# xipengwang/AprilSAM

Measured on NVIDIA H100. Metric: Gauss-Newton solves/sec (batch + incremental) on M3500 & 100k-pose graph, higher is better.
Workload: dtype f64

## Files before the change

aprilsam_b200/csrc/asam_kernels.cuh:

```cuda
#pragma once

#include <cuda_runtime.h>

#include <cstdint>

#include "asam_cuda.h"

#define ASAM_TR_FLAG (1 << 30)
#define ASAM_MAX_CACHED_CHILDREN 24

__device__ __forceinline__ double d_mod2pi(double v)
{
    const double twopi = 6.2831853071795862319959;
    const double pi = 3.141592653589793238462643383279502884196;
    double w = v + pi;
    return (w - twopi * floor(w / twopi)) - pi;
}

__device__ __forceinline__ void d_atb(const double *A, const double *B, double *C)
{
#pragma unroll
    for (int i = 0; i < 3; i++)
#pragma unroll
        for (int j = 0; j < 3; j++) {
// ... 1216 lines not shown
                    ok = 0;
                    break;
                }
            }
            __threadfence();
            *s_flag = ok;
        }
        __syncthreads();
        if (!*s_flag)
            return false;
        for (int e = tid; e < ASAM_TPB * ASAM_TPB; e += nt) {
            const int ii = e % ASAM_TPB, j = e / ASAM_TPB;
            D[e] = (ii >= j && ii < pb && j < pb) ? __ldcg(&F[(k0 + ii) + (size_t) (k0 + j) * ld]) : 0.0;
        }
        for (int e = tid; e < ASAM_TPB; e += nt)
            rdv[e] = e < pb ? __ldcg(&dinv[k0 + e]) : 0.0;
        __syncthreads();
        if (row)
            trsm_row(Li, D, rdv, pb, F + i + (size_t) k0 * ld, ld, Wnext ? Wnext + (size_t) i * ASAM_LDW : nullptr);
        return true;
    };

    {
        const int pb = min(ASAM_TPB, c);
        if (trow && tid == 0)
            t_mark = d_now();
        const int nchunk = (m + 1 + ASAM_TROWS - 1) / ASAM_TROWS;
        bool first = true;
        for (int ch = w; ch < nchunk || first; ch += G) {
            panel(0, pb, ch < nchunk ? ch * ASAM_TROWS : -1);
            first = false;
        }
        if (!team_barrier(tc, s_flag))
            return false;
        if (trow && tid == 0)
            t_panel += d_now() - t_mark;
        if (w == 0)
            writeback(0, pb);
    }
    int seq = 0;
    const bool pt_on = a.ptrace && s == a.ptrace_sn && w < 8 && tid == 0;
    for (int k0 = 0; k0 < c; k0 += ASAM_TPB) {
        unsigned long long *pt = (pt_on && k0 / ASAM_TPB < a.ptrace_panels) ? a.ptrace + ((size_t) (k0 / ASAM_TPB) * 8 + w) * 8 : nullptr;
        if (pt) {
            pt[0] = d_now();
            pt[1] = pt[2] = pt[3] = pt[0];
            pt[5] = (unsigned long long) m;
            pt[6] = (unsigned long long) G;
        }
        const int pb = min(ASAM_TPB, c - k0);
        const int kn0 = k0 + pb;
        const bool has_next = kn0 < c;
        const int pbn = has_next ? min(ASAM_TPB, c - kn0) : 0;
        const int ncrew = has_next ? 1 + (m - (kn0 + pbn) + 1 + ASAM_CROWS - 1) / ASAM_CROWS : 0;
        ++seq;
        if (w < ncrew) {
            if (trow && tid == 0)
                t_mark = d_now();
            if (w == 0) {
                __syncthreads();
                for (int e = tid; e < ASAM_TPB * ASAM_TPB; e += nt)
                    D[e] = 0.0;
                tile(k0, pb, kn0, pbn, kn0, pbn, D);
                if (pt)
                    pt[1] = d_now();
                diag_publish(kn0, pbn, seq);
                if (pt)
                    pt[2] = d_now();
            }
            if (v3) {
                for (int it = (w == 0 ? G : w); it < ncrew; it += G) {
                    const int rb0 = kn0 + pbn + (it - 1) * ASAM_CROWS;
                    tile_rm<2>(F, ld, Wbuf(k0 / ASAM_TPB), (pb + 3) & ~3, kn0, pbn, rb0, min(ASAM_CROWS, m - rb0 + 1), 2, Li, Li,
                               Lj3, mbar, mb_parity);
                    if (pt && w > 0 && it == w)
                        pt[1] = d_now();
                    if (!rows_solve_staged(kn0, pbn, rb0, seq, Wbuf(kn0 / ASAM_TPB)))
                        return false;
                }
            } else {
                for (int it = (w == 0 ? G : w); it < ncrew; it += G) {
                    const int rb0 = kn0 + pbn + (it - 1) * ASAM_CROWS;
                    tile(k0, pb, kn0, pbn, rb0, min(ASAM_CROWS, m - rb0 + 1), nullptr);
                }
                if (pt && w > 0)
                    pt[1] = d_now();
                for (int it = (w == 0 ? G : w); it < ncrew; it += G) {
                    const int rb0 = kn0 + pbn + (it - 1) * ASAM_CROWS;
                    if (!rows_solve(kn0, pbn, rb0, seq, nullptr))
                        return false;
                }
            }
            if (pt && w > 0)
                pt[2] = d_now();
            if (trow && tid == 0)
                t_panel += d_now() - t_mark;
        }

        const int j0 = kn0 + pbn;
        const int nfree = (G - ncrew >= 2) ? G - ncrew : G, wfree = (G - ncrew >= 2) ? w - ncrew : w;
        int n256 = 0;
        for (int cb0 = j0; cb0 < m; cb0 += ASAM_TCOLS)
            n256 += (m - cb0 + 1 + 255) / 256;
        const int TR = (n256 < 2 * nfree) ? 128 : 256;
        if (wfree >= 0) {
            int u = 0;
            for (int cb0 = j0; cb0 < m; cb0 += ASAM_TCOLS)
                for (int rb0 = cb0; rb0 <= m; rb0 += TR, ++u)
                    if (u % nfree == wfree)
                        tile(k0, pb, cb0, min(ASAM_TCOLS, m - cb0), rb0, min(TR, m - rb0 + 1), nullptr);
        }
        if (pt)
            pt[3] = d_now();
        if (!team_barrier(tc, s_flag))
            return false;
        if (pt) {
            pt[4] = d_now();
            pt[7] = (unsigned long long) ncrew;
        }
    }
    if (w == 0 && tid == 0)
        atomicExch(crew_bar, 0);

    if (trow && tid == 0) {
        trow[4] = d_now();
        trow[7] = (unsigned long long) (unsigned) m | (t_panel << 32);
    }
    if (w == 0) {
        for (int e = tid; e < c; e += nt)
            a.y[3 * (size_t) d.first + e] = __ldcg(&F[m + (size_t) e * ld]);
        __syncthreads();
        if (tid == 0 && d.parent >= 0) {
            __threadfence();
            atomicAdd(&a.arrive[d.parent], 1);
        }
    }
    team_leave(tc);
    __syncthreads();
    return true;
}

__device__ __forceinline__ void ticket_release(int *ticket, int *done)
{
    __syncthreads();
    if (threadIdx.x == 0) {
        __threadfence();
        if (atomicAdd(done, 1) == (int) gridDim.x - 1) {
            atomicExch(ticket, 0);
            atomicExch(done, 0);
        }
    }
}

__device__ bool cta_front(const FacArgs &a, const int t, const int s, const int nw, const asam_sn_desc_t &d, double *sm,
                          asam_sn_desc_t *s_cd, int *s_abort, unsigned long long tr0, const int keepw = 0)
{
    const int tid = threadIdx.x, nt = blockDim.x;
    const int lane = tid & 31, warp = tid >> 5, nwarps = nt >> 5;
    int *err = a.ctrl + 1;
    unsigned long long tr1 = 0, tr2 = 0, tr3 = 0, tr4 = 0, accA = 0, accB = 0;
    const int m = 3 * d.mb, c = 3 * d.cb, ld = ASAM_LD(m);
    const int *seg = a.ipool + d.seg;
    const int *children = seg + 2 * d.mb;
    const int *a_slot = children + d.ch_cnt;
    const int *a_rb = a_slot + d.a_cnt;
    const int *a_cb = a_rb + d.a_cnt;
    double *Fg = a.arena + d.f_off;
    const long long fsz = (long long) ld * m;
    const bool use_sm = fsz + (ld + 1) / 2 + 2 <= (long long) a.smem_doubles;
    double *F = use_sm ? sm : Fg;
    int *dmap = (int *) (sm + (use_sm ? fsz : 0));
    double *Pbuf = sm + (ld + 1) / 2 + 1;
    double *dinv = a.dinv + 3 * (size_t) d.first;

    if (use_sm) {
        for (int i = tid; i < (int) fsz; i += nt)
            F[i] = 0.0;
    } else {
        for (int j = warp; j < m; j += nwarps)
            for (int i = j + lane; i <= m; i += 32)
                F[i + (size_t) j * ld] = 0.0;
    }
    for (int e = tid; e < d.ch_cnt && e < ASAM_MAX_CACHED_CHILDREN; e += nt)
        s_cd[e] = a.sn[children[e]];
    __syncthreads();
    __shared__ int s_doff[ASAM_MAX_CACHED_CHILDREN + 1];
    bool dmap_ahead = false;
    if (use_sm && g_dmap_ahead && d.ch_cnt > 0 && d.ch_cnt <= ASAM_MAX_CACHED_CHILDREN) {
        if (tid == 0) {
            int o = 0;
            for (int e = 0; e < d.ch_cnt; e++) {
                s_doff[e] = o;
                o += 3 * (s_cd[e].mb - s_cd[e].cb) + 1;
            }
            s_doff[d.ch_cnt] = o;
        }
        __syncthreads();
        dmap_ahead = (long long) s_doff[d.ch_cnt] <= 2 * ((long long) a.smem_doubles - fsz) - 2;
        if (dmap_ahead)
            for (int ci = 0; ci < d.ch_cnt; ++ci) {
                const int cc = 3 * s_cd[ci].cb, cr = 3 * s_cd[ci].mb - cc;
                const int *crel = a.ipool + s_cd[ci].seg + s_cd[ci].mb;
                int *dm = dmap + s_doff[ci];
                for (int i = tid; i <= cr; i += nt)
                    dm[i] = (i < cr) ? 3 * crel[(cc + i) / 3] + (cc + i) % 3 : m;
            }
    }
    for (int e = tid; e < d.cb * 9; e += nt) {
        int k = e / 9, p = (e % 9) / 3, q = e % 3;
        if (p >= q)
            F[(3 * k + p) + (size_t) (3 * k + q) * ld] =
                a.Adiag[9 * (size_t) a.q2node[d.first + k] + q * 3 + p];
    }
    for (int e = tid; e < c; e += nt)
        F[m + (size_t) e * ld] = a.Bq[3 * (size_t) a.q2node[d.first + e / 3] + e % 3];
    for (int e = tid; e < d.a_cnt * 9; e += nt) {
        int i = e / 9, p = (e % 9) / 3, q = e % 3;
        const int rbf = a_rb[i];
        const int rb = rbf & ~ASAM_TR_FLAG;
        const int si = (rbf & ASAM_TR_FLAG) ? (p * 3 + q) : (q * 3 + p);
        F[(3 * rb + p) + (size_t) (3 * a_cb[i] + q) * ld] = a.Aoff[9 * (size_t) a_slot[i] + si];
    }
    if (a.trace && tid == 0)
        tr1 = d_now();

    if (nw > 0 && tid == 0) {
        SpinClock spins;
        while (ld_volatile(&a.arrive[s]) < nw) {
            __nanosleep(32);
            if (spin_over(spins, a.spin_limit) || ld_volatile(err) < 0) {
                atomicCAS(err, 0, -(1 + s));
                *s_abort = 1;
                break;
            }
        }
        a.arrive[s] = 0;
        __threadfence();
    }
    __syncthreads();
    if (*s_abort)
        return false;
    if (a.trace && tid == 0)
        tr2 = d_now();

    for (int ci = 0; ci < d.ch_cnt; ++ci) {
        const asam_sn_desc_t cd = ci < ASAM_MAX_CACHED_CHILDREN ? s_cd[ci] : a.sn[children[ci]];
        const int cm = 3 * cd.mb, cc = 3 * cd.cb, cr = cm - cc, cld = ASAM_LD(cm);
        const double *CF = a.arena + cd.f_off;
        const int *crel = a.ipool + cd.seg + cd.mb;
        if (dmap_ahead) {
            dmap = (int *) (sm + fsz) + s_doff[ci];
        } else {
            for (int i = tid; i <= cr; i += nt)
                dmap[i] = (i < cr) ? 3 * crel[(cc + i) / 3] + (cc + i) % 3 : m;
            __syncthreads();
        }
        if (use_sm && cr <= 159) {
            for (int j0 = warp; j0 < cr; j0 += 4 * nwarps) {
                double v[4][5];
#pragma unroll
                for (int q = 0; q < 4; q++) {
                    const int j = j0 + q * nwarps;
                    const double *ccol = CF + (size_t) (cc + min(j, cr - 1)) * cld + cc;
#pragma unroll
                    for (int u = 0; u < 5; u++) {
                        const int i = j + lane + 32 * u;
                        v[q][u] = (j < cr && i <= cr) ? __ldcg(ccol + i) : 0.0;
                    }
                }
#pragma unroll
                for (int q = 0; q < 4; q++) {
                    const int j = j0 + q * nwarps;
                    if (j < cr) {
                        double *fcol = F + (size_t) dmap[j] * ld;
#pragma unroll
                        for (int u = 0; u < 5; u++) {
                            const int i = j + lane + 32 * u;
                            if (i <= cr)
                                fcol[dmap[i]] += v[q][u];
                        }
                    }
                }
            }
        } else {
            for (int j = warp; j < cr; j += nwarps) {
                const double *ccol = CF + (size_t) (cc + j) * cld + cc;
                double *fcol = F + (size_t) dmap[j] * ld;
                for (int i0 = j + lane; i0 <= cr; i0 += 256) {
                    double v[8], dv[8];
                    int di[8];
#pragma unroll
                    for (int u = 0; u < 8; u++) {
                        const bool ok = i0 + 32 * u <= cr;
                        v[u] = ok ? __ldcg(ccol + i0 + 32 * u) : 0.0;
                        di[u] = ok ? dmap[i0 + 32 * u] : -1;
                    }
#pragma unroll
                    for (int u = 0; u < 8; u++)
                        dv[u] = di[u] >= 0 ? fcol[di[u]] : 0.0;
#pragma unroll
                    for (int u = 0; u < 8; u++)
                        if (di[u] >= 0)
                            fcol[di[u]] = dv[u] + v[u];
                }
            }
        }
        __syncthreads();
    }
    if (a.trace && tid == 0)
        tr3 = d_now();

    int kstart = 0;
    if (use_sm && keepw != 0) {
        const int keep = 3 * (keepw >> 16), m_old = 3 * (keepw & 0xffff), ld_old = ASAM_LD(m_old);
        if (keep > 0 && keep < c && m_old <= m && keep <= m_old) {
            for (int j = warp; j < keep; j += nwarps) {
                const double *oc = Fg + (size_t) j * ld_old;
                double *nc = F + (size_t) j * ld;
                for (int i = j + lane; i < m; i += 32)
                    nc[i] = i < m_old ? oc[i] : 0.0;
                if (lane == 0)
                    nc[m] = oc[m_old];
            }
            __syncthreads();
            if (a.smem_mma)
                trailing_update_mma(F, ld, F, ld, keep, keep, m, m);
            else
                trailing_update<2, 8>(F, ld, F, ld, keep, keep, m, m);
            __syncthreads();
            kstart = keep;
        }
    }
    if (use_sm) {
        const int pbw = a.pb_smem;
        for (int k0 = kstart; k0 < c; k0 += pbw) {
            const int pb = min(pbw, c - k0);
            double *P = F + (size_t) k0 * ld;
            unsigned long long ta = 0, tb = 0;
            if (a.trace && tid == 0)
                ta = d_now();
            panel_factor(P, ld, k0, pb, m, s, err, dinv);
            if (a.trace && tid == 0) {
                tb = d_now();
                accA += tb - ta;
            }
            const int n = m - (k0 + pb);
            if (a.smem_mma >= 2 && n > 0)
                trailing_update_mma(F, ld, P, ld, pb, k0 + pb, m, m);
            else if (n > 48)
                trailing_update<2, 8>(F, ld, P, ld, pb, k0 + pb, m, m);
            else
                trailing_update<1, 4>(F, ld, P, ld, pb, k0 + pb, m, m);
            __syncthreads();
        }
    } else {
        const int avail = a.smem_doubles - ((ld + 1) / 2 + 2);
        int PB = avail / ld;
        PB = PB > a.solo_pb ? a.solo_pb : PB;
        PB = PB >= ASAM_PB ? PB - (PB % ASAM_PB) : PB - (PB % 3);
        if (PB < 3) {
            if (tid == 0)
                atomicCAS(err, 0, -(1 + s));
            return false;
        }
        for (int k0 = 0; k0 < c; k0 += PB) {
            const int pbw = min(PB, c - k0);
            for (int p = warp; p < pbw; p += nwarps)
                for (int i = k0 + lane; i <= m; i += 32)
                    Pbuf[i + (size_t) p * ld] = F[i + (size_t) (k0 + p) * ld];
            __syncthreads();
            double *Cp = Pbuf - (size_t) k0 * ld;
            for (int k1 = 0; k1 < pbw; k1 += ASAM_PB) {
                const int pb = min(ASAM_PB, pbw - k1);
                panel_factor(Pbuf + (size_t) k1 * ld, ld, k0 + k1, pb, m, s, err, dinv);
                if (k1 + pb < pbw) {
                    trailing_update<2, 8>(Cp, ld, Pbuf + (size_t) k1 * ld, ld, pb, k0 + k1 + pb, k0 + pbw, m);
                    __syncthreads();
                }
            }
            for (int p = warp; p < pbw; p += nwarps)
                for (int i = k0 + lane; i <= m; i += 32)
                    F[i + (size_t) (k0 + p) * ld] = Pbuf[i + (size_t) p * ld];
            trailing_update<4, 8>(F, ld, Pbuf, ld, pbw, k0 + pbw, m, m);
            __syncthreads();
        }
    }
    if (a.trace && tid == 0)
        tr4 = d_now();

    if (use_sm) {
        for (int j = c + warp; j < m; j += nwarps)
            for (int i = j + lane; i <= m; i += 32)
                Fg[i + (size_t) j * ld] = F[i + (size_t) j * ld];
    }
    __syncthreads();
    if (tid == 0 && d.parent >= 0) {
        __threadfence();
        atomicAdd(&a.arrive[d.parent], 1);
    }
    for (int e = tid; e < c; e += nt)
        a.y[3 * (size_t) d.first + e] = F[m + (size_t) e * ld];
    if (use_sm) {
        for (int j = warp; j < c; j += nwarps)
            for (int i = j + lane; i <= m; i += 32)
                Fg[i + (size_t) j * ld] = F[i + (size_t) j * ld];
    }
    __syncthreads();
    if (tid == 0) {
        if (a.trace) {
            unsigned smid;
            asm volatile("mov.u32 %0, %%smid;" : "=r"(smid));
            unsigned long long *tr = a.trace + 8 * (size_t) t;
            tr[0] = tr0; tr[1] = tr1; tr[2] = tr2; tr[3] = tr3; tr[4] = tr4; tr[5] = d_now();
            (void) smid;
            tr[6] = (unsigned long long) s | (accB << 32);
            tr[7] = (unsigned long long) (unsigned) m | (accA << 32);
        }
    }
    __syncthreads();
    return true;
}

__global__ void __launch_bounds__(256, 1) k_factor(FacArgs a)
{
    extern __shared__ __align__(16) double sm[];
    __shared__ int s_task, s_abort;
    __shared__ asam_sn_desc_t s_cd[ASAM_MAX_CACHED_CHILDREN];
    __shared__ __align__(8) unsigned long long s_mbar;
    const int tid = threadIdx.x;
    unsigned mb_parity = 0;
    if (tid == 0)
        mbar_init(&s_mbar, 1);
    __syncthreads();
    for (;;) {
        if (tid == 0) {
            s_task = atomicAdd(&a.ctrl[0], 1);
            s_abort = 0;
        }
        __syncthreads();
        const int t = s_task;
        if (t >= a.ntasks)
            break;
        unsigned long long tr0 = 0;
        if (a.trace && tid == 0)
            tr0 = d_now();
        const int s = a.tasks[t];
        const int nwp = a.nwait[t];
        const int nw = nwp & 0xffff, tw = (nwp >> 16) & 0xff, tG = (nwp >> 24) & 0x7f;
        const asam_sn_desc_t d = a.sn[s];
        if (tG >= 1) {
            unsigned long long *trow = (a.trace && tw == 0) ? a.trace + 8 * (size_t) t : nullptr;
            if (trow && tid == 0) {
                trow[0] = tr0; trow[1] = tr0;
            }
            if (!team_front(a, d, s, nw, tw, tG, sm, &s_abort, trow, &s_mbar, mb_parity))
                break;
            if (a.trace && tid == 0) {
                unsigned long long *tr = a.trace + 8 * (size_t) t;
                if (tw == 0) {
                    tr[5] = d_now();
                    tr[6] = (unsigned long long) s | ((unsigned long long) tG << 32);
                } else {
                    tr[0] = tr0; tr[1] = tr0; tr[2] = tr0; tr[3] = tr0; tr[4] = d_now(); tr[5] = tr[4];
                    tr[6] = (unsigned long long) s | ((unsigned long long) tG << 32);
                    tr[7] = (unsigned long long) (unsigned) (3 * d.mb);
                }
            }
            __syncthreads();
            continue;
        }
        if (!cta_front(a, t, s, nw, d, sm, s_cd, &s_abort, tr0, a.keep ? a.keep[t] : 0))
            break;
    }
    ticket_release(&a.ctrl[0], &a.ctrl[3]);
}

#define ASAM_LEAF_M 63
#define ASAM_LEAF_WARPS 7
#define ASAM_LEAF_STRIDE (ASAM_LD(ASAM_LEAF_M) * ASAM_LEAF_M + ASAM_LEAF_M / 2 + 2)

struct LeafArgs {
    const asam_sn_desc_t *sn;
    const int *ipool;
    double *arena;
    const double *Adiag, *Aoff, *Bq;
    const int *q2node;
    double *y;
    double *dinv;
    int *arrive;
    const int *tasks;
    int ntasks;
    int *ctrl;
    long long spin_limit;
};

__global__ void __launch_bounds__(32 * ASAM_LEAF_WARPS, 1) k_factor_leaf(LeafArgs a)
{
    extern __shared__ __align__(16) double sm[];
    const int lane = threadIdx.x & 31, warp = threadIdx.x >> 5;
    double *F = sm + (size_t) warp * ASAM_LEAF_STRIDE;
    int *dmap = (int *) (F + ASAM_LD(ASAM_LEAF_M) * ASAM_LEAF_M);
    int *err = a.ctrl + 1;
    for (;;) {
        int t = 0;
        if (lane == 0)
            t = atomicAdd(&a.ctrl[5], 1);
        t = __shfl_sync(0xffffffffu, t, 0);
        if (t >= a.ntasks)
            break;
        const int s = a.tasks[t];
        const asam_sn_desc_t d = a.sn[s];
        const int m = 3 * d.mb, c = 3 * d.cb, ld = ASAM_LD(m);
        if (m > ASAM_LEAF_M) {
            if (lane == 0)
                atomicCAS(err, 0, -(1 + s));
            break;
        }
        const int *seg = a.ipool + d.seg;
        const int *children = seg + 2 * d.mb;
        const int *a_slot = children + d.ch_cnt;
        const int *a_rb = a_slot + d.a_cnt;
        const int *a_cb = a_rb + d.a_cnt;
        double *Fg = a.arena + d.f_off;
        const int fsz = ld * m;

        for (int i = lane; i < fsz; i += 32)
            F[i] = 0.0;
        __syncwarp();
        for (int e = lane; e < d.cb * 9; e += 32) {
            int k = e / 9, p = (e % 9) / 3, q = e % 3;
            if (p >= q)
                F[(3 * k + p) + (3 * k + q) * ld] = a.Adiag[9 * (size_t) a.q2node[d.first + k] + q * 3 + p];
        }
        for (int e = lane; e < c; e += 32)
            F[m + e * ld] = a.Bq[3 * (size_t) a.q2node[d.first + e / 3] + e % 3];
        for (int e = lane; e < d.a_cnt * 9; e += 32) {
// ... 699 lines not shown
```

aprilsam_b200/host/plan.c:

```c
#define _POSIX_C_SOURCE 200809L
#include <math.h>
#include <stdio.h>
#include <stdlib.h>
#include <string.h>
#include <time.h>

#include "asam_host.h"

static double g_plan_prof[8];
static double g_build_prof[8];
static double pp_now(void)
{
    struct timespec ts;
    clock_gettime(CLOCK_MONOTONIC, &ts);
    return ts.tv_sec * 1e3 + ts.tv_nsec * 1e-6;
}
void asam_dbg_plan_profile(double *out, int reset)
{
    memcpy(out, g_plan_prof, sizeof(g_plan_prof));
    if (reset)
        memset(g_plan_prof, 0, sizeof(g_plan_prof));
}
void asam_dbg_build_profile(double *out, int reset)
{
// ... 292 lines not shown
            asam_set_error("plan: supernode %d has rows below but no parent", s);
            return 1;
        }
        return 0;
    }
    const ivec_t *pr = &pl->snh[P].rows;
    int j = 0;
    for (int k = cb; k < h->rows.n; k++) {
        int v = h->rows.p[k];
        while (j < pr->n && pr->p[j] < v)
            j++;
        if (j >= pr->n || pr->p[j] != v) {
            asam_set_error("plan: row %d of supernode %d missing in parent %d", v, s, P);
            return 1;
        }
        h->rel.p[k] = j;
    }
    return 0;
}

static void emit_segment(plan_t *pl, int s, ivec_t *buf, int64_t base)
{
    sn_host_t *h = &pl->snh[s];
    asam_sn_desc_t *d = &pl->desc[s];
    d->seg = (int32_t) (base + buf->n);
    d->mb = h->rows.n;
    d->ch_cnt = h->children.n;
    d->a_cnt = h->a_slot.n;
    int need = buf->n + 2 * h->rows.n + h->children.n + 3 * h->a_slot.n;
    ivec_reserve(buf, need);
    const ivec_t *parts[6] = { &h->rows, &h->rel, &h->children, &h->a_slot, &h->a_rb, &h->a_cb };
    const int lens[6] = { h->rows.n, h->rows.n, h->children.n, h->a_slot.n, h->a_slot.n, h->a_slot.n };
    for (int i = 0; i < 6; i++) {
        if (lens[i] > 0)
            memcpy(buf->p + buf->n, parts[i]->p, sizeof(int) * (size_t) lens[i]);
        buf->n += lens[i];
    }
}

static int front_fits_smem(int mb)
{
    int64_t m = 3 * (int64_t) mb;
    return (int64_t) ASAM_LD(m) * m + (ASAM_LD(m) + 1) / 2 + 2 <= 25600;
}

static int solo_max_m(void)
{
    static int v = -1;
    if (v < 0) {
        const char *e = getenv("ASAM_SOLO_MAX_M");
        v = e ? atoi(e) : ASAM_SOLO_MAX_M_DEFAULT;
    }
    return v;
}

static int team_size(int mb, int cb, int cap)
{
    int64_t m = 3 * (int64_t) mb, c = 3 * (int64_t) cb;
    if (front_fits_smem(mb) || m <= solo_max_m())
        return 1;
    int64_t j0 = c < 48 ? c : 48, tiles = 0;
    for (int64_t cb0 = j0; cb0 < m; cb0 += 64)
        tiles += (m - cb0 + 1 + 255) / 256;
    int64_t chunks = 1 + (m - j0 + 1 + 127) / 128;
    static int tpw = 0;
    if (tpw == 0) {
        const char *e = getenv("ASAM_TILES_PER_WORKER");
        tpw = e && atoi(e) > 0 ? atoi(e) : ASAM_TILES_PER_WORKER;
    }
    int G = (int) ((tiles + tpw - 1) / tpw + chunks);
    if (cap < 2)
        cap = 2;
    if (cap > 120)
        cap = 120;
    if (G < 2)
        G = 2;
    if (G > cap)
        G = cap;
    return G;
}

static inline int pack_nwait(int nw, int w, int G)
{
    if (nw < 0 || nw > 0xffff || w < 0 || w > 0xff || G < 0 || G > 0x7f)
        asam_fatal("plan: task word overflow (%d children in one launch, worker %d of %d): hub supernodes with more "
                   "than 65535 re-factored children are not supported", nw, w, G);
    return (nw & 0xffff) | (w << 16) | (G << 24);
}

static int plan_team_cap(const plan_t *pl) { return pl->max_team > 0 ? pl->max_team : 120; }

static int64_t front_doubles(int mb)
{
    int64_t m = 3 * (int64_t) mb;
    return (int64_t) ASAM_LD(m) * m + (front_fits_smem(mb) ? 0 : 2 * (m + 2) * 52);
}

static double sn_work(const asam_sn_desc_t *d)
{
    double m = 3.0 * d->mb, c = 3.0 * d->cb;
    return c * m * m + 3.0e4;
}

void plan_work(const plan_t *pl, const int *tasks, int ntasks, double *step_work, int *step_fronts, double *batch_work,
               int *batch_fronts)
{
    double sw = 0.0, bw = 0.0;
    int sf = 0, last = -1;
    for (int t = 0; t < ntasks; t++) {
        if (tasks[t] == last)
            continue;
        last = tasks[t];
        sw += sn_work(&pl->desc[last]);
        sf++;
    }
    for (int s = 0; s < pl->nsn; s++)
        bw += sn_work(&pl->desc[s]);
    *step_work = sw;
    *step_fronts = sf;
    *batch_work = bw;
    *batch_fronts = pl->nsn;
}

typedef struct {
    double key;
    int id;
} sn_key_t;

static int cmp_key_desc(const void *a, const void *b)
{
    const sn_key_t *x = a, *y = b;
    if (x->key != y->key)
        return x->key > y->key ? -1 : 1;
    return (x->id > y->id) - (x->id < y->id);
}

static double team_model[5] = { 21.5, 24.4, 11.6, 0.041, 0.0 };
static void team_model_init(void)
{
    static int done = 0;
    if (done)
        return;
    done = 1;
    const char *e = getenv("ASAM_TEAM_MODEL");
    if (e)
        sscanf(e, "%lf,%lf,%lf,%lf,%lf", &team_model[0], &team_model[1], &team_model[2], &team_model[3], &team_model[4]);
}

static double front_lat_us(const plan_t *pl, int s, int g)
{
    const double m = 3.0 * pl->desc[s].mb, c = 3.0 * pl->desc[s].cb;
    if (m <= 48)
        return 2.0 + 0.1 * c;
    if (front_fits_smem(pl->desc[s].mb) || g < 1)
        return 3.8 + 0.121 * m + 0.105 * c + 0.00508 * c * m;
    double tiles = 0.0, crew = 0.0;
    const int npan = (int) ceil(c / 48.0);
    for (int k = 0; k < npan; k++) {
        const double r = m - 48.0 * (k + 1) > 0 ? m - 48.0 * (k + 1) : 0.0;
        tiles += r * r / 2.0 / (256.0 * 64.0);
        crew += 1.0 + ceil(r / 128.0);
    }
    return team_model[0] * npan + team_model[1] * tiles / g + team_model[2] * crew / g + team_model[3] * m +
           team_model[4] * m * m / 1024.0 / g;
}

typedef struct {
    double key;
    int id;
} hp_t;

static void hp_push(hp_t *h, int *n, double key, int id, int maxheap)
{
    int i = (*n)++;
    h[i].key = key;
    h[i].id = id;
    while (i > 0) {
        int p = (i - 1) / 2;
        int better = maxheap ? (h[i].key > h[p].key || (h[i].key == h[p].key && h[i].id < h[p].id))
                             : (h[i].key < h[p].key || (h[i].key == h[p].key && h[i].id < h[p].id));
        if (!better)
            break;
        hp_t t = h[p]; h[p] = h[i]; h[i] = t;
        i = p;
    }
}

static hp_t hp_pop(hp_t *h, int *n, int maxheap)
{
    hp_t top = h[0];
    h[0] = h[--(*n)];
    int i = 0;
    for (;;) {
        int l = 2 * i + 1, r = l + 1, b = i;
        for (int c = l; c <= r; c++) {
            if (c >= *n)
                break;
            int better = maxheap ? (h[c].key > h[b].key || (h[c].key == h[b].key && h[c].id < h[b].id))
                                 : (h[c].key < h[b].key || (h[c].key == h[b].key && h[c].id < h[b].id));
            if (better)
                b = c;
        }
        if (b == i)
            break;
        hp_t t = h[b]; h[b] = h[i]; h[i] = t;
        i = b;
    }
    return top;
}

static int sim_order(const plan_t *pl, const char *in, const int *G_of, const double *lat, const double *prio, int P, int *out)
{
    const int nsn = pl->nsn;
    int *pending = calloc((size_t) nsn + 1, sizeof(int));
    hp_t *ready = malloc(sizeof(hp_t) * (size_t) (nsn + 1)), *events = malloc(sizeof(hp_t) * (size_t) (nsn + 1));
    int nready = 0, nev = 0, nout = 0, free_cta = P;
    for (int s = 0; s < nsn; s++)
        if (in[s] && pl->desc[s].parent >= 0 && in[pl->desc[s].parent])
            pending[pl->desc[s].parent]++;
    for (int s = 0; s < nsn; s++)
        if (in[s] && pending[s] == 0)
            hp_push(ready, &nready, prio[s], s, 1);
    double now = 0.0;
    for (;;) {
        while (nready > 0) {
            int s = ready[0].id, g = G_of[s] < 0 ? 1 : (G_of[s] > P ? P : G_of[s]);
            if (g > free_cta && nev > 0)
                break;
            hp_pop(ready, &nready, 1);
            out[nout++] = s;
            free_cta -= g < free_cta ? g : free_cta;
            hp_push(events, &nev, now + lat[s], s, 0);
        }
        if (nev == 0)
            break;
        hp_t e = hp_pop(events, &nev, 0);
        now = e.key;
        {
            int s = e.id, g = G_of[s] < 0 ? 1 : (G_of[s] > P ? P : G_of[s]);
            free_cta += g;
            if (free_cta > P)
                free_cta = P;
            int par = pl->desc[s].parent;
            if (par >= 0 && in[par] && --pending[par] == 0)
                hp_push(ready, &nready, prio[par], par, 1);
        }
    }
    free(pending);
    free(ready);
    free(events);
    return nout;
}

static void build_schedule(plan_t *pl)
{
    const int nsn = pl->nsn, W = pl->world > 1 ? pl->world : 1, me = pl->world > 1 ? pl->rank : 0;
    free(pl->tasks); free(pl->nwait); free(pl->btasks); free(pl->leaf_tasks);
    free(pl->top_tasks); free(pl->top_nwait);
    free(pl->shard_owner); free(pl->shard_off); free(pl->shard_cnt); free(pl->shard_q0); free(pl->shard_qn);
    pl->top_tasks = pl->top_nwait = pl->shard_owner = pl->shard_q0 = pl->shard_qn = NULL;
    pl->shard_off = pl->shard_cnt = NULL;
    pl->n_top = pl->n_top_sn = pl->n_shards = 0;

    int *owner = malloc(sizeof(int) * (size_t) (nsn + 1));
    for (int s = 0; s < nsn; s++)
        owner[s] = 0;
    if (W > 1 && nsn > 0) {
        double *sub = malloc(sizeof(double) * (size_t) nsn);
        for (int s = 0; s < nsn; s++)
            sub[s] = sn_work(&pl->desc[s]);
        for (int s = 0; s < nsn; s++)
            if (pl->desc[s].parent >= 0)
                sub[pl->desc[s].parent] += sub[s];
        int *fr = malloc(sizeof(int) * (size_t) (nsn + 1)), nfr = 0;
        double total = 0.0;
        for (int s = 0; s < nsn; s++)
            if (pl->desc[s].parent < 0) {
                fr[nfr++] = s;
                total += sub[s];
            }
        for (int s = 0; s < nsn; s++)
            owner[s] = -2;
        const int max_shards = 16 * W;
        const double shard_tol = getenv("ASAM_SHARD_TOL") ? atof(getenv("ASAM_SHARD_TOL")) : ASAM_SHARD_TOL_DEFAULT;
        double *load = malloc(sizeof(double) * (size_t) W);
        for (;;) {
            for (int i = 1; i < nfr; i++) {
                int v = fr[i], j = i - 1;
                while (j >= 0 && (sub[fr[j]] < sub[v] || (sub[fr[j]] == sub[v] && fr[j] > v))) {
                    fr[j + 1] = fr[j];
                    j--;
                }
                fr[j + 1] = v;
            }
            for (int r = 0; r < W; r++)
                load[r] = 0.0;
            double shard_sum = 0.0;
            for (int i = 0; i < nfr; i++) {
                int best = 0;
                for (int r = 1; r < W; r++)
                    if (load[r] < load[best])
                        best = r;
                load[best] += sub[fr[i]];
                shard_sum += sub[fr[i]];
            }
            double mx = 0.0;
            for (int r = 0; r < W; r++)
                if (load[r] > mx)
                    mx = load[r];
            int h = fr[0];
            if (nfr >= W && mx <= shard_tol * shard_sum / W)
                break;
            if (nfr >= max_shards || pl->snh[h].children.n == 0)
                break;
            owner[h] = -1;
            fr[0] = fr[nfr - 1];
            nfr--;
            for (int c = 0; c < pl->snh[h].children.n; c++)
                fr[nfr++] = pl->snh[h].children.p[c];
        }
        for (int r = 0; r < W; r++)
            load[r] = 0.0;
        pl->n_shards = nfr;
        pl->shard_owner = malloc(sizeof(int) * (size_t) (nfr + 1));
        pl->shard_off = malloc(sizeof(int64_t) * (size_t) (nfr + 1));
        pl->shard_cnt = malloc(sizeof(int64_t) * (size_t) (nfr + 1));
        pl->shard_q0 = malloc(sizeof(int) * (size_t) (nfr + 1));
        pl->shard_qn = malloc(sizeof(int) * (size_t) (nfr + 1));
        int *npose = calloc((size_t) nsn + 1, sizeof(int));
        for (int s = 0; s < nsn; s++) {
            npose[s] += pl->desc[s].cb;
            if (pl->desc[s].parent >= 0)
                npose[pl->desc[s].parent] += npose[s];
        }
        for (int i = 0; i < nfr; i++) {
            int best = 0, s = fr[i];
            for (int r = 1; r < W; r++)
                if (load[r] < load[best])
                    best = r;
            load[best] += sub[s];
            owner[s] = best;
            const asam_sn_desc_t *d = &pl->desc[s];
            int64_t m = 3 * (int64_t) d->mb, c = 3 * (int64_t) d->cb, ld = ASAM_LD(m);
            pl->shard_owner[i] = best;
            pl->shard_off[i] = d->f_off + c * ld;
            pl->shard_cnt[i] = (m - c) * ld;
            pl->shard_qn[i] = npose[s];
            pl->shard_q0[i] = d->first + d->cb - npose[s];
        }
        for (int s = nsn - 1; s >= 0; s--)
            if (owner[s] == -2)
                owner[s] = pl->desc[s].parent >= 0 ? owner[pl->desc[s].parent] : -1;
        free(npose);
        free(load);
        free(fr);
        free(sub);
    }

    char *leaf = calloc((size_t) nsn + 1, 1);
    int n_leaf_all = 0;
    const int leaf_max = leaf_max_m_for(nsn);
    for (int s = 0; s < nsn; s++) {
        int ok = 3 * pl->desc[s].mb <= leaf_max;
        for (int c = 0; ok && c < pl->snh[s].children.n; c++)
            ok = leaf[pl->snh[s].children.p[c]];
        leaf[s] = (char) ok;
        n_leaf_all += ok;
    }
    if (n_leaf_all < ASAM_LEAF_MIN_COUNT)
        memset(leaf, 0, (size_t) nsn);
    free(pl->bs_leaf);
    pl->bs_leaf = calloc((size_t) pl->sn_cap + 1, 1);
    for (int s = 0; s < nsn; s++) {
        int ok = 3 * pl->desc[s].cb <= ASAM_BSLEAF_MAX && 3 * (pl->desc[s].mb - pl->desc[s].cb) <= ASAM_BSLEAF_MAX;
        for (int c = 0; ok && c < pl->snh[s].children.n; c++)
            ok = pl->bs_leaf[pl->snh[s].children.p[c]];
        pl->bs_leaf[s] = (char) ok;
    }

    int *byl = malloc(sizeof(int) * (size_t) (nsn + 1));
    int order_mode = 0;
    int *bylv = malloc(sizeof(int) * (size_t) (nsn + 1));
    {
        int *cnt = calloc((size_t) pl->n_levels + 2, sizeof(int));
        for (int s = 0; s < nsn; s++)
            cnt[pl->desc[s].level + 1]++;
        for (int l = 0; l < pl->n_levels; l++)
            cnt[l + 1] += cnt[l];
        for (int s = 0; s < nsn; s++)
            bylv[cnt[pl->desc[s].level]++] = s;
        free(cnt);
    }
    {
        const char *eo = getenv("ASAM_TASK_ORDER");
        if (eo && strcmp(eo, "level") == 0) {
            memcpy(byl, bylv, sizeof(int) * (size_t) nsn);
        } else {
            order_mode = (eo && strcmp(eo, "cp") == 0) ? 1 : ((eo && strcmp(eo, "sim") == 0) ? 2 : 3);
        }
    }

    int *G_of = malloc(sizeof(int) * (size_t) (nsn + 1));
    {
        int64_t *want = calloc((size_t) pl->n_levels + 1, sizeof(int64_t));
        for (int s = 0; s < nsn; s++) {
            G_of[s] = (owner[s] == me || owner[s] == -1) && !leaf[s] ? team_size(pl->desc[s].mb, pl->desc[s].cb, plan_team_cap(pl)) : 1;
            if (G_of[s] > 1)
                want[pl->desc[s].level] += G_of[s];
        }
        int64_t room = ASAM_TEAM_ROOM < plan_team_cap(pl) ? ASAM_TEAM_ROOM : plan_team_cap(pl);
        const char *er = getenv("ASAM_TEAM_ROOM");
        if (er && atoi(er) > 0)
            room = atoi(er);
        int gmin = 1;
        const char *em = getenv("ASAM_TEAM_MIN");
        if (em && atoi(em) >= 1)
            gmin = atoi(em);
        for (int s = 0; s < nsn; s++) {
            int64_t w = want[pl->desc[s].level];
            if (G_of[s] > 1 && w > room) {
                int g = (int) ((int64_t) G_of[s] * room / w);
                G_of[s] = g < gmin ? gmin : g;
            }
            if (G_of[s] == 1 && !leaf[s] && !front_fits_smem(pl->desc[s].mb) && 3 * pl->desc[s].mb > solo_max_m())
                G_of[s] = -1;
        }
        free(want);
    }
    if (order_mode != 0) {
        double *lat_us = malloc(sizeof(double) * (size_t) (nsn + 1)), *up_us = malloc(sizeof(double) * (size_t) (nsn + 1));
        double work = 0.0, chain = 0.0;
        team_model_init();
        for (int s = nsn - 1; s >= 0; s--) {
            const int g = G_of[s] < 0 ? 1 : G_of[s];
            const double lat = front_lat_us(pl, s, g);
            lat_us[s] = lat;
            up_us[s] = lat + (pl->desc[s].parent >= 0 ? up_us[pl->desc[s].parent] : 0.0);
            if ((owner[s] == me || owner[s] == -1) && !leaf[s])
                work += lat * g;
            if (up_us[s] > chain)
                chain = up_us[s];
        }
        const int P = pl->n_cta > 0 ? pl->n_cta : 132;
        const int use_sim = order_mode == 2 || (order_mode == 3 && work / P > 0.5 * chain);
        {
            sn_key_t *keys = malloc(sizeof(sn_key_t) * (size_t) (nsn + 1));
            for (int s = 0; s < nsn; s++) {
                keys[s].key = up_us[s];
                keys[s].id = s;
            }
            qsort(keys, (size_t) nsn, sizeof(sn_key_t), cmp_key_desc);
            for (int k = 0; k < nsn; k++)
                byl[k] = keys[k].id;
            free(keys);
        }
        if (use_sim) {
            char *in = calloc((size_t) nsn + 1, 1);
            int *ord = malloc(sizeof(int) * (size_t) (nsn + 1)), *pos_of = malloc(sizeof(int) * (size_t) (nsn + 1));
            int n1, n2;
            for (int s = 0; s < nsn; s++)
                in[s] = owner[s] == me && !leaf[s];
            n1 = sim_order(pl, in, G_of, lat_us, up_us, P, ord);
            for (int s = 0; s < nsn; s++)
                in[s] = owner[s] == -1;
            n2 = sim_order(pl, in, G_of, lat_us, up_us, P, ord + n1);
            for (int s = 0; s < nsn; s++)
                pos_of[s] = -1;
            for (int k = 0; k < n1 + n2; k++)
                pos_of[ord[k]] = k;
            int *nb = malloc(sizeof(int) * (size_t) (nsn + 1)), k2 = 0;
            for (int k = 0; k < n1 + n2; k++)
                nb[k2++] = ord[k];
            for (int k = 0; k < nsn; k++)
                if (pos_of[byl[k]] < 0)
                    nb[k2++] = byl[k];
            memcpy(byl, nb, sizeof(int) * (size_t) nsn);
            free(nb);
            free(in);
            free(ord);
            free(pos_of);
        }
        free(lat_us);
        free(up_us);
    }

    int bs_split = 1;
    {
        const char *eb = getenv("ASAM_BS_SPLIT");
        if (eb)
            bs_split = atoi(eb) != 0;
    }
    pl->bt_split = 0;
#define BS_NBLK(s_) ((bs_split && !pl->bs_leaf[s_] && 3 * pl->desc[s_].cb > 96 && pl->nsn < (1 << 24)) ? (3 * pl->desc[s_].cb + 95) / 96 : 1)
    int64_t n_local = 0, n_top = 0;
    int n_leaf = 0, n_main_sn = 0, n_top_sn = 0, n_bsl = 0, n_top_bt = 0;
    for (int s = 0; s < nsn; s++)
        n_bsl += owner[s] == me && pl->bs_leaf[s];
    if (n_bsl < ASAM_BSLEAF_MIN_COUNT) {
        memset(pl->bs_leaf, 0, (size_t) nsn);
        n_bsl = 0;
    }
    for (int s = 0; s < nsn; s++) {
        if (owner[s] == me) {
            if (leaf[s])
                n_leaf++;
            else
                n_local += G_of[s] < 0 ? 1 : G_of[s];
            if (!pl->bs_leaf[s])
                n_main_sn += BS_NBLK(s);
        } else if (owner[s] == -1) {
            n_top += G_of[s] < 0 ? 1 : G_of[s];
            n_top_sn++;
            n_top_bt += BS_NBLK(s);
        }
    }
    pl->ntasks = (int) n_local;
    pl->tasks = malloc(sizeof(int) * (size_t) (n_local + 1));
    pl->nwait = malloc(sizeof(int) * (size_t) (n_local + 1));
    pl->n_leaf = n_leaf;
    pl->leaf_tasks = malloc(sizeof(int) * (size_t) (n_leaf + 1));
    pl->n_top = (int) n_top;
    pl->n_top_sn = n_top_sn;
    pl->top_tasks = malloc(sizeof(int) * (size_t) (n_top + 1));
    pl->top_nwait = malloc(sizeof(int) * (size_t) (n_top + 1));
    pl->n_bs_leaf = n_bsl;
    pl->n_btasks = n_top_bt + n_main_sn + n_bsl;
    pl->btasks = malloc(sizeof(int) * (size_t) (pl->n_btasks + 1));
    {
        const char *eb = getenv("ASAM_BS_ORDER");
        if (!(eb && strcmp(eb, "level") == 0) && nsn > 0) {
            double *down = calloc((size_t) nsn, sizeof(double));
            sn_key_t *keys = malloc(sizeof(sn_key_t) * (size_t) nsn);
            for (int s = 0; s < nsn; s++) {
                if (!pl->bs_leaf[s])
                    down[s] += 5.0 + 0.17 * 3.0 * pl->desc[s].cb + 0.01 * 3.0 * pl->desc[s].mb;
                else
                    down[s] += 1e-3 * (pl->desc[s].level + 1);
                const int par = pl->desc[s].parent;
                if (par >= 0 && down[s] > down[par])
                    down[par] = down[s];
                keys[s].key = down[s];
                keys[s].id = s;
            }
            qsort(keys, (size_t) nsn, sizeof(sn_key_t), cmp_key_desc);
            for (int k = 0; k < nsn; k++)
                bylv[nsn - 1 - k] = keys[k].id;
            free(keys);
            free(down);
        }
    }
    int t = 0, tl = 0, tt = 0;
    int bt = n_top_bt - 1, bm = n_top_bt + n_main_sn - 1, bl = pl->n_btasks - 1;
    for (int k = 0; k < nsn; k++) {
        int s = bylv[k];
        if (owner[s] == -1) {
            const int nb = BS_NBLK(s);
            for (int b = 0; b < nb; b++)
                pl->btasks[bt--] = nb > 1 ? (s | ((b + 1) << 24)) : s;
            pl->bt_split |= nb > 1;
        } else if (owner[s] == me) {
            if (pl->bs_leaf[s]) {
                pl->btasks[bl--] = s;
            } else {
                const int nb = BS_NBLK(s);
                for (int b = 0; b < nb; b++)
                    pl->btasks[bm--] = nb > 1 ? (s | ((b + 1) << 24)) : s;
                pl->bt_split |= nb > 1;
            }
        }
    }
    for (int k = 0; k < nsn; k++) {
        int s = byl[k];
        if (owner[s] == -1) {
            int nw = 0;
            for (int c = 0; c < pl->snh[s].children.n; c++)
                nw += owner[pl->snh[s].children.p[c]] == -1;
            int G = G_of[s] < 0 ? 1 : G_of[s];
            for (int w = 0; w < G; w++, tt++) {
                pl->top_tasks[tt] = s;
                pl->top_nwait[tt] = pack_nwait(nw, w, G > 1 ? G : (G_of[s] < 0 ? 1 : 0));
            }
            continue;
        }
        if (owner[s] != me)
            continue;
        if (leaf[s]) {
            pl->leaf_tasks[tl++] = s;
            continue;
// ... 850 lines not shown
```

Baseline: 128.7.

## Use DMMA tensor-core updates and padded panel buffer in solo out-of-smem fronts

Result: faster. 136.6, median of 6 (+6.2%).

```diff
diff --git a/aprilsam_b200/csrc/asam_kernels.cuh b/aprilsam_b200/csrc/asam_kernels.cuh
--- a/aprilsam_b200/csrc/asam_kernels.cuh
+++ b/aprilsam_b200/csrc/asam_kernels.cuh
@@ -1392,6 +1392,91 @@
     }
 }
 
+__device__ __forceinline__ void solo_copy(double *dst, const int ldd, const double *src, const int lds, const int nr2,
+                                          const int ncol)
+{
+    const int n = nr2 * ncol, nt = blockDim.x;
+    for (int e0 = threadIdx.x; e0 < n; e0 += 8 * nt) {
+        double2 v[8];
+#pragma unroll
+        for (int u = 0; u < 8; u++) {
+            const int e = e0 + u * nt, p = e / nr2, r = e - p * nr2;
+            if (e < n)
+                v[u] = *(const double2 *) (src + 2 * r + (size_t) p * lds);
+        }
+#pragma unroll
+        for (int u = 0; u < 8; u++) {
+            const int e = e0 + u * nt, p = e / nr2, r = e - p * nr2;
+            if (e < n)
+                *(double2 *) (dst + 2 * r + (size_t) p * ldd) = v[u];
+        }
+    }
+}
+
+__device__ __forceinline__ void solo_tile_next(int &jb, int &ib, const int m, int n)
+{
+    for (; n > 0 && jb < m; --n) {
+        ib += 32;
+        if (ib > m) {
+            jb += 8;
+            ib = jb;
+        }
+    }
+}
+
+__device__ __noinline__ void solo_update(double *F, const int ld, const double *P, const int ldp, const int pb,
+                                         const int j0, const int m)
+{
+    const int lane = threadIdx.x & 31, warp = threadIdx.x >> 5, nwarps = blockDim.x >> 5;
+    const int g = lane >> 2, t = lane & 3;
+    auto load_c = [&](const int jb, const int ib, double (&v)[4][2]) {
+#pragma unroll
+        for (int mt = 0; mt < 4; mt++)
+#pragma unroll
+            for (int e = 0; e < 2; e++) {
+                const int i = ib + 8 * mt + g, j = jb + 2 * t + e;
+                v[mt][e] = (jb < m && i <= m && j < m && i >= j) ? F[i + (size_t) j * ld] : 0.0;
+            }
+    };
+    int jb = j0, ib = j0;
+    solo_tile_next(jb, ib, m, warp);
+    double cv[4][2];
+    load_c(jb, ib, cv);
+    while (jb < m) {
+        int jn = jb, in = ib;
+        solo_tile_next(jn, in, m, nwarps);
+        double cn[4][2];
+        load_c(jn, in, cn);
+        double acc[4][2];
+#pragma unroll
+        for (int mt = 0; mt < 4; mt++)
+            acc[mt][0] = acc[mt][1] = 0.0;
+        const bool jok = jb + g < m;
+        for (int kk = 0; kk < pb; kk += 4) {
+            const bool kok = kk + t < pb;
+            const size_t koff = (size_t) (kk + t) * ldp;
+            const double bv = (kok && jok) ? P[(jb + g) + koff] : 0.0;
+#pragma unroll
+            for (int mt = 0; mt < 4; mt++) {
+                const int row = ib + 8 * mt + g;
+                const double av = (kok && row <= m) ? -P[row + koff] : 0.0;
+                dmma_8x8x4(acc[mt][0], acc[mt][1], av, bv);
+            }
+        }
+#pragma unroll
+        for (int mt = 0; mt < 4; mt++)
+#pragma unroll
+            for (int e = 0; e < 2; e++) {
+                const int i = ib + 8 * mt + g, j = jb + 2 * t + e;
+                if (i <= m && j < m && i >= j)
+                    F[i + (size_t) j * ld] = cv[mt][e] + acc[mt][e];
+                cv[mt][e] = cn[mt][e];
+            }
+        jb = jn;
+        ib = in;
+    }
+}
+
 __device__ bool cta_front(const FacArgs &a, const int t, const int s, const int nw, const asam_sn_desc_t &d, double *sm,
                           asam_sn_desc_t *s_cd, int *s_abort, unsigned long long tr0, const int keepw = 0)
 {
@@ -1410,7 +1495,7 @@
     const bool use_sm = fsz + (ld + 1) / 2 + 2 <= (long long) a.smem_doubles;
     double *F = use_sm ? sm : Fg;
     int *dmap = (int *) (sm + (use_sm ? fsz : 0));
-    double *Pbuf = sm + (ld + 1) / 2 + 1;
+    const int pboff = ((ld + 1) / 2 + 2) & ~1;
     double *dinv = a.dinv + 3 * (size_t) d.first;
 
     if (use_sm) {
@@ -1594,8 +1679,9 @@
             __syncthreads();
         }
     } else {
-        const int avail = a.smem_doubles - ((ld + 1) / 2 + 2);
-        int PB = avail / ld;
+        double *Pbuf = sm + pboff;
+        const int ldp = ((m + 2) & ~15) + (((m + 2) & 15) <= 4 ? 4 : 20);
+        int PB = (a.smem_doubles - pboff) / ldp;
         PB = PB > a.solo_pb ? a.solo_pb : PB;
         PB = PB >= ASAM_PB ? PB - (PB % ASAM_PB) : PB - (PB % 3);
         if (PB < 3) {
@@ -1605,23 +1691,21 @@
         }
         for (int k0 = 0; k0 < c; k0 += PB) {
             const int pbw = min(PB, c - k0);
-            for (int p = warp; p < pbw; p += nwarps)
-                for (int i = k0 + lane; i <= m; i += 32)
-                    Pbuf[i + (size_t) p * ld] = F[i + (size_t) (k0 + p) * ld];
+            const int kr = k0 & ~1, nr2 = (m - kr + 2) >> 1;
+            double *Pst = Pbuf - kr;
+            solo_copy(Pbuf, ldp, F + kr + (size_t) k0 * ld, ld, nr2, pbw);
             __syncthreads();
-            double *Cp = Pbuf - (size_t) k0 * ld;
+            double *Cp = Pst - (size_t) k0 * ldp;
             for (int k1 = 0; k1 < pbw; k1 += ASAM_PB) {
                 const int pb = min(ASAM_PB, pbw - k1);
-                panel_factor(Pbuf + (size_t) k1 * ld, ld, k0 + k1, pb, m, s, err, dinv);
+                panel_factor(Pst + (size_t) k1 * ldp, ldp, k0 + k1, pb, m, s, err, dinv);
                 if (k1 + pb < pbw) {
-                    trailing_update<2, 8>(Cp, ld, Pbuf + (size_t) k1 * ld, ld, pb, k0 + k1 + pb, k0 + pbw, m);
+                    trailing_update_mma(Cp, ldp, Pst + (size_t) k1 * ldp, ldp, pb, k0 + k1 + pb, k0 + pbw, m);
                     __syncthreads();
                 }
             }
-            for (int p = warp; p < pbw; p += nwarps)
-                for (int i = k0 + lane; i <= m; i += 32)
-                    F[i + (size_t) (k0 + p) * ld] = Pbuf[i + (size_t) p * ld];
-            trailing_update<4, 8>(F, ld, Pbuf, ld, pbw, k0 + pbw, m, m);
+            solo_copy(F + kr + (size_t) k0 * ld, ld, Pbuf, ldp, nr2, pbw);
+            solo_update(F, ld, Pst, ldp, pbw, k0 + pbw, m);
             __syncthreads();
         }
     }
diff --git a/aprilsam_b200/host/plan.c b/aprilsam_b200/host/plan.c
--- a/aprilsam_b200/host/plan.c
+++ b/aprilsam_b200/host/plan.c
@@ -468,8 +468,10 @@
     const double m = 3.0 * pl->desc[s].mb, c = 3.0 * pl->desc[s].cb;
     if (m <= 48)
         return 2.0 + 0.1 * c;
-    if (front_fits_smem(pl->desc[s].mb) || g < 1)
+    if (front_fits_smem(pl->desc[s].mb))
         return 3.8 + 0.121 * m + 0.105 * c + 0.00508 * c * m;
+    if (g < 1)
+        return 0.119 * m + 0.00631 * c * m;
     double tiles = 0.0, crew = 0.0;
     const int npan = (int) ceil(c / 48.0);
     for (int k = 0; k < npan; k++) {
@@ -728,7 +730,7 @@
         const char *er = getenv("ASAM_TEAM_ROOM");
         if (er && atoi(er) > 0)
             room = atoi(er);
-        int gmin = 1;
+        int gmin = 0;
         const char *em = getenv("ASAM_TEAM_MIN");
         if (em && atoi(em) >= 1)
             gmin = atoi(em);
@@ -736,10 +738,9 @@
             int64_t w = want[pl->desc[s].level];
             if (G_of[s] > 1 && w > room) {
                 int g = (int) ((int64_t) G_of[s] * room / w);
-                G_of[s] = g < gmin ? gmin : g;
-            }
-            if (G_of[s] == 1 && !leaf[s] && !front_fits_smem(pl->desc[s].mb) && 3 * pl->desc[s].mb > solo_max_m())
-                G_of[s] = -1;
+                g = g < gmin ? gmin : g;
+                G_of[s] = g >= 2 ? g : (gmin == 1 ? -1 : 1);
+            }
         }
         free(want);
     }
@@ -749,7 +750,7 @@
         team_model_init();
         for (int s = nsn - 1; s >= 0; s--) {
             const int g = G_of[s] < 0 ? 1 : G_of[s];
-            const double lat = front_lat_us(pl, s, g);
+            const double lat = front_lat_us(pl, s, G_of[s] == 1 ? 0 : g);
             lat_us[s] = lat;
             up_us[s] = lat + (pl->desc[s].parent >= 0 ? up_us[pl->desc[s].parent] : 0.0);
             if ((owner[s] == me || owner[s] == -1) && !leaf[s])
```
